# zhouyou-gu/sig-sdp-mmw

Hardware: AMD Instinct MI355X
Metric: mmw_iterations_per_sec (higher is better)
Workload: dtype f32

## Files before the change

### sig_sdp_mmw_amd/csrc/kernels_mfma.h

```cpp
#pragma once
#include "kernels_expm.h"

namespace mmw {

typedef short mf_s4 __attribute__((ext_vector_type(4)));
typedef short mf_s8 __attribute__((ext_vector_type(8)));
typedef __bf16 mf_bf8 __attribute__((ext_vector_type(8)));
typedef float mf_f16 __attribute__((ext_vector_type(16)));

__device__ __forceinline__ unsigned short bf16_rn(float x) { return __builtin_bit_cast(unsigned short, (__bf16)x); }
__device__ __forceinline__ float bf16_f32(unsigned short h) { return __uint_as_float((unsigned)h << 16); }
__device__ __forceinline__ unsigned split_bf16(float x) {
    const unsigned short hi = bf16_rn(x);
    const unsigned short lo = bf16_rn(x - bf16_f32(hi));
    return ((unsigned)hi << 16) | (unsigned)lo;
}

__global__ __launch_bounds__(BLOCK) void k_split_planes(size_t n4, const float4* __restrict__ src, uint2* __restrict__ hi, uint2* __restrict__ lo) {
    for (size_t o = (size_t)blockIdx.x * BLOCK + threadIdx.x; o < n4; o += (size_t)gridDim.x * BLOCK) {
        const float4 x = src[o];
        const unsigned a = split_bf16(x.x), b = split_bf16(x.y), c = split_bf16(x.z), d = split_bf16(x.w);
        hi[o] = make_uint2((a >> 16) | (b & 0xFFFF0000u), (c >> 16) | (d & 0xFFFF0000u));
        lo[o] = make_uint2((a & 0xFFFFu) | (b << 16), (c & 0xFFFFu) | (d << 16));
    }
}

constexpr double SDM_FX = 1099511627776.0;
constexpr int MF_KROWS = 16;
constexpr int MF_UNION_ROWS = 640;
constexpr int MF_KPAD = 4;
struct MfmaDev {
    int nb;
    const int* desc;
    const int* un_fixed;
    const int* order;
    const int* kbase;
    const unsigned* afrag;
};
struct MfEpi {
    const float* F = nullptr;
    const float* X2 = nullptr;
    float c3 = 0.f;
    unsigned short* out_planes = nullptr;
    unsigned short* y_planes = nullptr;
    long long* dfx = nullptr;
    double* tr_part = nullptr;
};
template <int MT, int GT, int KC, int PL = 2, int AP = 2> constexpr int mf_chunk_bytes() { return KC * (1024 * PL * GT + 1024 * AP * MT); }
template <int MT, int GT, int KC, int NB, int PL = 2, int AP = 2> constexpr int mf_lds_bytes() { return MF_UNION_ROWS * 4 + 64 * 4 + NB * mf_chunk_bytes<MT, GT, KC, PL, AP>(); }
constexpr bool mf_first(int mode) { return mode == SPMM_FIRST || mode == SPMM_FIRST16; }
constexpr int mf_planes(int mode) { return mf_first(mode) ? 1 : 2; }
constexpr int mf_apieces(int mode) { return mode == SPMM_FIRST16 ? 1 : 2; }
typedef _Float16 mf_h8 __attribute__((ext_vector_type(8)));
constexpr float MF_F16_SCALE = 1048576.0f;
__device__ __forceinline__ unsigned short f16_rn(float x) { return __builtin_bit_cast(unsigned short, (_Float16)x); }
__device__ __forceinline__ float f16_f32(unsigned short h) { return (float)__builtin_bit_cast(_Float16, h); }
__device__ __forceinline__ unsigned split_f16_scaled(float x) {
    const float xs = x * MF_F16_SCALE;
    const unsigned short hi = f16_rn(xs);
    const unsigned short lo = f16_rn(xs - f16_f32(hi));
    return ((unsigned)hi << 16) | (unsigned)lo;
}
__device__ __forceinline__ size_t mf_pos16(int w) {
    const int j = (w & 3) + 4 * ((w >> 8) & 1), lane = (w >> 2) & 63;
    return ((size_t)(w >> 9) * 64 + lane) * 8 + j;
}
__global__ __launch_bounds__(BLOCK) void k_plane_f16(size_t n4, const float4* __restrict__ src, uint2* __restrict__ dst) {
    for (size_t o = (size_t)blockIdx.x * BLOCK + threadIdx.x; o < n4; o += (size_t)gridDim.x * BLOCK) {
        const float4 x = src[o];
        dst[o] = make_uint2((unsigned)f16_rn(x.x) | ((unsigned)f16_rn(x.y) << 16), (unsigned)f16_rn(x.z) | ((unsigned)f16_rn(x.w) << 16));
    }
}


__device__ __forceinline__ void mf_wait_vmcnt(int n) {
    switch (n) {
#define MMW_W(N) case N: asm volatile("s_waitcnt vmcnt(" #N ")" ::: "memory"); break;
        MMW_W(0) MMW_W(1) MMW_W(2) MMW_W(3) MMW_W(4) MMW_W(5) MMW_W(6) MMW_W(7) MMW_W(8) MMW_W(9) MMW_W(10) MMW_W(11) MMW_W(12)
        MMW_W(13) MMW_W(14) MMW_W(15) MMW_W(16) MMW_W(17) MMW_W(18) MMW_W(19) MMW_W(20) MMW_W(21) MMW_W(22) MMW_W(23) MMW_W(24)
        MMW_W(25) MMW_W(26) MMW_W(27) MMW_W(28) MMW_W(29) MMW_W(30) MMW_W(31) MMW_W(32) MMW_W(33) MMW_W(34) MMW_W(35) MMW_W(36)
        MMW_W(37) MMW_W(38) MMW_W(39) MMW_W(40) MMW_W(41) MMW_W(42) MMW_W(43) MMW_W(44) MMW_W(45) MMW_W(46) MMW_W(47) MMW_W(48)
#undef MMW_W
        default: asm volatile("s_waitcnt vmcnt(0)" ::: "memory"); break;
    }
}

__device__ __forceinline__ int mf_div(int n, int d, float rd) { (void)d; return (int)(((float)n + 0.5f) * rd); }
__device__ __forceinline__ void mf_dma16(const char* src, unsigned lds) {
    asm volatile("s_mov_b32 m0, %1\n\ts_nop 0\n\tglobal_load_lds_dwordx4 %0, off" : : "v"(src), "s"(lds) : "memory", "m0");
}

template <int MODE, int MT, int NT, int NW, int MS, int KC, int NB>
__global__ __launch_bounds__(NW * 64)
void k_spmm_mfma(MfmaDev M, int Dpad, size_t plane_bytes, const char* __restrict__ Upl, const float* __restrict__ U,
                 float* __restrict__ Out, double ascale_d, double shift_d, double* __restrict__ partial, double* __restrict__ partial_o2,
                 const ExpmPlan* __restrict__ plan, int step, int* __restrict__ viol, unsigned long long* __restrict__ stamps, MfEpi E) {
    static_assert(MODE == SPMM_PLAIN || MODE == SPMM_LANCZOS || MODE == SPMM_AXPBY || mf_first(MODE), "the matrix-core SpMM has the plain, the Lanczos, the AXPBY and the first-order epilogue");
    static_assert(MF_KPAD % KC == 0, "the fragment image pads a block's k-steps to whole chunks");
    constexpr bool F16 = mf_first(MODE);
    constexpr bool A16 = MODE == SPMM_FIRST16;
    constexpr int AP = mf_apieces(MODE), AB = 1024 * AP;
    unsigned long long tk0 = 0, tk1 = 0, acc_wait = 0, acc_issue = 0, acc_comp = 0, t_pro = 0;
    if (stamps) tk0 = __builtin_amdgcn_s_memtime();
    typedef __attribute__((address_space(3))) void* lds_vp;
    typedef const __attribute__((address_space(1))) void* glb_vp;
    constexpr int THREADS = NW * 64;
    bool shifted = false;
    if (plan) {
        if (MODE == SPMM_LANCZOS) {
            if (step > plan_steps(plan, step - 1)) return;
            shifted = plan->apost != 0 && partial_o2 != nullptr;
            if (shifted) shift_d = plan->mu;
        } else if (F16) {
            shift_d = plan->mu;
        } else if (step > plan->m) return;
        if (!(A16 ? plan->f16a_ok : (F16 ? plan->f16_ok : plan->mfma_ok)) && viol && blockIdx.x == 0 && blockIdx.y == 0 && threadIdx.x == 0) atomicOr(viol, VIOL_OPERANDS);
    }
    const float ascale = (float)ascale_d, shift = (float)shift_d;
    static_assert(NW % MS == 0 && MT % MS == 0, "row tiles and waves split evenly");
    constexpr int NWN = NW / MS;
    constexpr int MTW = MT / MS;
    constexpr int GT = NWN * NT;
    constexpr int PL = mf_planes(MODE);
    constexpr int CHUNK = mf_chunk_bytes<MT, GT, KC, PL, AP>();
    constexpr int B1 = 1024 * PL * GT;
    constexpr int A_OFF = KC * B1;
    extern __shared__ __attribute__((aligned(16))) char smem_raw[];
    int* un_l = reinterpret_cast<int*>(smem_raw);
    int* orow_l = reinterpret_cast<int*>(smem_raw + MF_UNION_ROWS * 4);
    char* bufs = smem_raw + MF_UNION_ROWS * 4 + 64 * 4;
    const unsigned bufs_l = (unsigned)(size_t)(lds_vp)bufs;

    const int per = (M.nb + 7) >> 3;
    const int rb = (blockIdx.x & 7) * per + (blockIdx.x >> 3);
    if (rb >= M.nb) return;
    const int col0 = blockIdx.y * (GT * 32);
    const int ng = min(GT, (Dpad - col0) >> 5);
    const int spr = ng * 4;
    const int* dsc = M.desc + (size_t)rb * 8;
    const int q0 = dsc[0], nrows = dsc[1];
    const int kb = M.kbase[rb];
    const int KS = M.kbase[rb + 1] - kb;
    const int NC = KS / KC;
    const int lane = threadIdx.x & 63;
    const int wv = __builtin_amdgcn_readfirstlane(threadIdx.x >> 6);
    const int wm = wv / NWN, wn = wv - wm * NWN;

    for (int i = threadIdx.x; i < KS * MF_KROWS; i += THREADS) un_l[i] = M.un_fixed[(size_t)rb * MF_UNION_ROWS + i];
    if ((int)threadIdx.x < 64) orow_l[threadIdx.x] = (int)threadIdx.x < nrows ? M.order[q0 + threadIdx.x] : -1;

    const int rmode = (ng & 3) == 0 ? 2 : ((ng & 3) == 2 ? 1 : 0);
    auto rot = [&](int q) { return rmode == 2 ? q : (rmode == 1 ? (q >> 1) : 0); };

    constexpr int NJ = (KC * (PL * GT + AP * MT) + NW - 1) / NW;
    const int nB1 = PL * ng, nP1 = nB1 + AP * MT, nI = KC * nP1;
    const int cw = wv < nI ? (nI - wv + NW - 1) / NW : 0;
    const char* pbase[NJ];
    unsigned pmul[NJ];
    int prow[NJ], pdst[NJ];
    const unsigned pitch = (unsigned)Dpad * 2u;
    const char* afr = reinterpret_cast<const char*>(M.afrag) + (size_t)kb * (AB * MT);
    const float rP1 = 1.0f / (float)nP1, rspr = 1.0f / (float)spr;
#pragma unroll
    for (int j = 0; j < NJ; ++j) {
        const int i = wv + NW * j;
        const int kk = mf_div(i, nP1, rP1), i1 = i - kk * nP1;
        pbase[j] = Upl;
        pmul[j] = 0;
        prow[j] = 0;
        pdst[j] = 0;
        if (i < nI && i1 < nB1) {
            const int slot = i1 * 64 + lane;
            const int p = (PL == 2 && slot >= MF_KROWS * spr) ? 1 : 0, rem = slot - p * (MF_KROWS * spr);
            const int r = mf_div(rem, spr, rspr), t = rem - r * spr;
            int G = (t >> 2) - rot(r & 3);
            if (G < 0) G += ng;
            pbase[j] = Upl + ((size_t)p * plane_bytes + (size_t)col0 * 2u + (size_t)(G * 4 + (t & 3)) * 16u);
            pmul[j] = pitch;
            prow[j] = kk * MF_KROWS + r;
            pdst[j] = kk * B1 + i1 * 1024;
        } else if (i < nI) {
            pbase[j] = afr + (kk * (AB * MT) + (i1 - nB1) * 1024 + lane * 16);
            pdst[j] = A_OFF + kk * (AB * MT) + (i1 - nB1) * 1024;
        }
        pdst[j] = __builtin_amdgcn_readfirstlane(pdst[j]);
    }
    auto issue = [&](int c) {
        const unsigned dst_l = bufs_l + (unsigned)((c % NB) * CHUNK);
        const unsigned astep = (unsigned)c * (unsigned)(KC * AB * MT);
#pragma unroll
        for (int j = 0; j < NJ; ++j) {
            if (j < cw) {
                const char* src = pbase[j] + ((size_t)(unsigned)un_l[c * (KC * MF_KROWS) + prow[j]] * pmul[j] + (pmul[j] ? 0u : astep));
                mf_dma16(src, dst_l + (unsigned)pdst[j]);
            }
        }
    };

    const int g16 = lane >> 4, l16 = lane & 15, tq = l16 >> 2, tp = l16 & 3;
    unsigned rbase[NT];
    bool tile_on[NT];
#pragma unroll
    for (int i = 0; i < NT; ++i) {
        const int G = wn * NT + i;
        tile_on[i] = G < ng;
        int Gp = (tile_on[i] ? G : 0) + rot(tq);
        if (Gp >= ng) Gp -= ng;
        rbase[i] = (unsigned)((8 * (g16 >> 1) + tq) * spr * 16 + Gp * 64 + (g16 & 1) * 32 + tp * 8);
    }
    const unsigned row4 = (unsigned)(4 * spr * 16), plane_l = (unsigned)(MF_KROWS * spr * 16);

    mf_f16 acc[MTW][NT];
#pragma unroll
    for (int m = 0; m < MTW; ++m)
#pragma unroll
        for (int i = 0; i < NT; ++i)
#pragma unroll
            for (int v = 0; v < 16; ++v) acc[m][i][v] = 0.f;

    __syncthreads();
#pragma unroll
    for (int c = 0; c < NB - 1; ++c)
        if (c < NC) issue(c);
    if (stamps) { tk1 = __builtin_amdgcn_s_memtime(); t_pro = tk1 - tk0; }
    for (int c = 0; c < NC; ++c) {
        const int younger = min(NC - 1 - c, NB - 2);
        mf_wait_vmcnt(cw * younger);
        __builtin_amdgcn_s_barrier();
        if (stamps) { const unsigned long long t = __builtin_amdgcn_s_memtime(); acc_wait += t - tk1; tk1 = t; }
        if (c + NB - 1 < NC) issue(c + NB - 1);
        if (stamps) { const unsigned long long t = __builtin_amdgcn_s_memtime(); acc_issue += t - tk1; tk1 = t; }
        const char* cb = bufs + (c % NB) * CHUNK;
#pragma unroll
        for (int kk = 0; kk < KC; ++kk) {
            const char* bb = cb + kk * B1;
            mf_s8 ahi[MTW], alo[MTW];
#pragma unroll
            for (int m = 0; m < MTW; ++m) {
                const char* af = cb + A_OFF + (kk * MT + wm * MTW + m) * AB + lane * 16;
                const uint4 a0 = *reinterpret_cast<const uint4*>(af);
                if constexpr (A16) {
                    ahi[m] = __builtin_bit_cast(mf_s8, a0);
                    alo[m] = ahi[m];
                    continue;
                }
                const uint4 a1 = *reinterpret_cast<const uint4*>(af + 1024);
                const unsigned w[8] = {a0.x, a0.y, a0.z, a0.w, a1.x, a1.y, a1.z, a1.w};
                unsigned h[4], l[4];
#pragma unroll
                for (int i = 0; i < 4; ++i) {
                    h[i] = __builtin_amdgcn_perm(w[2 * i + 1], w[2 * i], 0x07060302u);
                    l[i] = __builtin_amdgcn_perm(w[2 * i + 1], w[2 * i], 0x05040100u);
                }
                const uint4 hv = make_uint4(h[0], h[1], h[2], h[3]), lv = make_uint4(l[0], l[1], l[2], l[3]);
                ahi[m] = __builtin_bit_cast(mf_s8, hv);
                alo[m] = __builtin_bit_cast(mf_s8, lv);
            }
#pragma unroll
            for (int i = 0; i < NT; ++i) {
                typedef __attribute__((address_space(3))) mf_s4* lp;
                const char* p0 = bb + rbase[i];
                const mf_s4 h0 = __builtin_amdgcn_ds_read_tr16_b64_v4i16((lp)(p0));
                const mf_s4 h1 = __builtin_amdgcn_ds_read_tr16_b64_v4i16((lp)(p0 + row4));
                if constexpr (F16) {
                    const mf_s8 bh = {h0[0], h0[1], h0[2], h0[3], h1[0], h1[1], h1[2], h1[3]};
#pragma unroll
                    for (int m = 0; m < MTW; ++m) {
                        if constexpr (!A16) acc[m][i] = __builtin_amdgcn_mfma_f32_32x32x16_f16(__builtin_bit_cast(mf_h8, alo[m]), __builtin_bit_cast(mf_h8, bh), acc[m][i], 0, 0, 0);
                        acc[m][i] = __builtin_amdgcn_mfma_f32_32x32x16_f16(__builtin_bit_cast(mf_h8, ahi[m]), __builtin_bit_cast(mf_h8, bh), acc[m][i], 0, 0, 0);
                    }
                } else {
                    const mf_s4 l0 = __builtin_amdgcn_ds_read_tr16_b64_v4i16((lp)(p0 + plane_l));
                    const mf_s4 l1 = __builtin_amdgcn_ds_read_tr16_b64_v4i16((lp)(p0 + plane_l + row4));
                    const mf_s8 bhi = {h0[0], h0[1], h0[2], h0[3], h1[0], h1[1], h1[2], h1[3]};
                    const mf_s8 blo = {l0[0], l0[1], l0[2], l0[3], l1[0], l1[1], l1[2], l1[3]};
#pragma unroll
                    for (int m = 0; m < MTW; ++m) {
                        acc[m][i] = __builtin_amdgcn_mfma_f32_32x32x16_bf16(__builtin_bit_cast(mf_bf8, alo[m]), __builtin_bit_cast(mf_bf8, bhi), acc[m][i], 0, 0, 0);
                        acc[m][i] = __builtin_amdgcn_mfma_f32_32x32x16_bf16(__builtin_bit_cast(mf_bf8, ahi[m]), __builtin_bit_cast(mf_bf8, blo), acc[m][i], 0, 0, 0);
                        acc[m][i] = __builtin_amdgcn_mfma_f32_32x32x16_bf16(__builtin_bit_cast(mf_bf8, ahi[m]), __builtin_bit_cast(mf_bf8, bhi), acc[m][i], 0, 0, 0);
                    }
                }
            }
        }
        if (stamps) { const unsigned long long t = __builtin_amdgcn_s_memtime(); acc_comp += t - tk1; tk1 = t; }
    }

    if constexpr (F16) {
        const int h2 = lane >> 5, cl = lane & 31;
        const float emu = Out ? (float)exp(shift_d) : 1.f;
        float* red = reinterpret_cast<float*>(bufs);
        float* rowred = red + MS * GT * 32;
        static_assert((MS * GT * 32 + NWN * 32 * MT) * 4 <= NB * CHUNK, "the epilogue's reductions fit into the chunk buffers");
        float rn[MTW][16], d2t[NT];
#pragma unroll
        for (int m = 0; m < MTW; ++m)
#pragma unroll
            for (int v = 0; v < 16; ++v) rn[m][v] = 0.f;
#pragma unroll
        for (int i = 0; i < NT; ++i) {
            if (!tile_on[i]) continue;
            const int col = col0 + (wn * NT + i) * 32 + cl;
            float dot2 = 0.f;
#pragma unroll
            for (int m = 0; m < MTW; ++m) {
                int rows[16];
                float u[16], yy[16];
#pragma unroll
                for (int v = 0; v < 16; ++v) rows[v] = orow_l[32 * (wm * MTW + m) + (v & 3) + 8 * (v >> 2) + 4 * h2];
#pragma unroll
                for (int v = 0; v < 16; ++v) u[v] = U[(size_t)max(rows[v], 0) * Dpad + col];
#pragma unroll
                for (int v = 0; v < 16; ++v) {
                    const float o = ascale * acc[m][i][v] - shift * u[v];
                    const float y = u[v] + o;
                    yy[v] = 0.f;
                    if (rows[v] >= 0) {
                        dot2 += o * o;
                        yy[v] = y * y;
                        if (Out) Out[(size_t)rows[v] * Dpad + col] = y * emu;
                    }
                    const unsigned w = split_bf16(y);
                    const unsigned wp = dpp_u32<DPP_QUAD_XOR1>(w);
                    if (rows[v] >= 0) {
                        const unsigned val = (cl & 1) ? ((wp & 0xFFFFu) | (w << 16)) : ((w >> 16) | (wp & 0xFFFF0000u));
                        unsigned short* g = E.y_planes + (size_t)rows[v] * Dpad * 2 + (size_t)(col >> 5) * 64 + ((cl & 1) ? 32 : 0) + (col & 30);
                        *reinterpret_cast<unsigned*>(g) = val;
                    }
                }
#pragma unroll
                for (int v = 0; v < 16; ++v) rn[m][v] += group_sum(yy[v], 32);
            }
            float a, b;
            rows32(dot2, a, b);
            d2t[i] = a + b;
        }
        __syncthreads();
#pragma unroll
        for (int i = 0; i < NT; ++i)
            if (tile_on[i] && h2 == 0) red[(wm * GT + wn * NT + i) * 32 + cl] = d2t[i];
        if (cl == 0) {
#pragma unroll
            for (int m = 0; m < MTW; ++m)
#pragma unroll
                for (int v = 0; v < 16; ++v) rowred[wn * (32 * MT) + 32 * (wm * MTW + m) + (v & 3) + 8 * (v >> 2) + 4 * h2] = rn[m][v];
        }
        __syncthreads();
        for (int t = threadIdx.x; t < ng * 32; t += THREADS) {
            float d2 = 0.f;
#pragma unroll
            for (int g = 0; g < MS; ++g) d2 += red[g * GT * 32 + t];
            partial_o2[(size_t)rb * Dpad + col0 + t] = (double)d2;
        }
        if (wv == 0) {
            double s = 0.0;
            if (lane < nrows) {
                float f = 0.f;
#pragma unroll
                for (int g = 0; g < NWN; ++g) f += rowred[g * (32 * MT) + lane];
                s = (double)f;
                atomicAdd(reinterpret_cast<unsigned long long*>(E.dfx) + orow_l[lane], (unsigned long long)__double2ll_rn(s * SDM_FX));
            }
            s = wave_sum(s);
            if (lane == 0) E.tr_part[(size_t)blockIdx.y * gridDim.x + blockIdx.x] = s;
        }
        if (stamps && lane == 0) {
            const unsigned long long te = __builtin_amdgcn_s_memtime();
            unsigned long long* o = stamps + ((size_t)(blockIdx.y * gridDim.x + blockIdx.x) * NW + wv) * 8;
            o[0] = t_pro; o[1] = acc_wait; o[2] = acc_issue; o[3] = acc_comp; o[4] = te - tk0; o[5] = (unsigned long long)NC; o[6] = tk0; o[7] = te - tk1;
        }
        return;
    }
    const int h2 = lane >> 5, cl = lane & 31;
#pragma unroll
    for (int i = 0; i < NT; ++i) {
        if (!tile_on[i]) continue;
        const int col = col0 + (wn * NT + i) * 32 + cl;
        float dot = 0.f, dot2 = 0.f;
#pragma unroll
        for (int m = 0; m < MTW; ++m) {
            int rows[16];
            float u[16];
#pragma unroll
            for (int v = 0; v < 16; ++v) rows[v] = orow_l[32 * (wm * MTW + m) + (v & 3) + 8 * (v >> 2) + 4 * h2];
            float x2[16];
            if (MODE == SPMM_LANCZOS) {
#pragma unroll
                for (int v = 0; v < 16; ++v) u[v] = U[(size_t)max(rows[v], 0) * Dpad + col];
            }
            if (MODE == SPMM_AXPBY) {
#pragma unroll
                for (int v = 0; v < 16; ++v) {
                    u[v] = E.F[(size_t)max(rows[v], 0) * Dpad + col];
                    x2[v] = E.X2[(size_t)max(rows[v], 0) * Dpad + col];
                }
            }
#pragma unroll
            for (int v = 0; v < 16; ++v) {
                float o;
                if (MODE == SPMM_LANCZOS) {
                    o = ascale * acc[m][i][v] - shift * u[v];
                    if (rows[v] >= 0) {
                        dot += u[v] * o;
                        dot2 += o * o;
                    }
                } else if (MODE == SPMM_AXPBY) {
                    o = ascale * acc[m][i][v] + shift * u[v] + E.c3 * x2[v];
                } else {
                    o = ascale * acc[m][i][v];
                }
                if (rows[v] >= 0) {
                    const size_t at = (size_t)rows[v] * Dpad + col;
                    Out[at] = o;
                    if (MODE != SPMM_LANCZOS && E.out_planes) {
                        const unsigned w = split_bf16(o);
                        E.out_planes[at] = (unsigned short)(w >> 16);
                        *reinterpret_cast<unsigned short*>(reinterpret_cast<char*>(E.out_planes) + plane_bytes + at * 2) = (unsigned short)(w & 0xFFFFu);
                    }
                }
            }
        }
        if (MODE == SPMM_LANCZOS) {
            float a, b;
            rows32(dot, a, b);
            const float d1 = a + b;
            rows32(dot2, a, b);
            const float d2 = a + b;
            if (MS == 1) {
                if (h2 == 0) {
                    partial[(size_t)rb * Dpad + col] = (double)d1;
                    if (shifted) partial_o2[(size_t)rb * Dpad + col] = (double)d2;
                }
            } else if (h2 == 0) {
                float* red = reinterpret_cast<float*>(bufs);
                red[((wm * GT + wn * NT + i) * 32 + cl) * 2] = d1;
                red[((wm * GT + wn * NT + i) * 32 + cl) * 2 + 1] = d2;
            }
        }
    }
    if (MODE == SPMM_LANCZOS && MS > 1) {
        __syncthreads();
        const float* red = reinterpret_cast<const float*>(bufs);
        for (int t = threadIdx.x; t < ng * 32; t += THREADS) {
            float d1 = 0.f, d2 = 0.f;
#pragma unroll
            for (int g = 0; g < MS; ++g) {
                d1 += red[((g * GT) * 32 + t) * 2];
                d2 += red[((g * GT) * 32 + t) * 2 + 1];
            }
            partial[(size_t)rb * Dpad + col0 + t] = (double)d1;
            if (shifted) partial_o2[(size_t)rb * Dpad + col0 + t] = (double)d2;
        }
    }
    if (stamps && lane == 0) {
        const unsigned long long te = __builtin_amdgcn_s_memtime();
        unsigned long long* o = stamps + ((size_t)(blockIdx.y * gridDim.x + blockIdx.x) * NW + wv) * 8;
        o[0] = t_pro; o[1] = acc_wait; o[2] = acc_issue; o[3] = acc_comp; o[4] = te - tk0; o[5] = (unsigned long long)NC; o[6] = tk0; o[7] = te - tk1;
    }
}


struct SdMfmaDev {
    const int* tbase;
    const int* tptr;
    const unsigned short* trc;
    const unsigned short* tmask;
    int nedges;
};
constexpr int SDM_GT = 4;
constexpr int SDM_KC = 2;
template <int MT> constexpr int sdm_rows() { return 32 * MT + 32 * SDM_GT; }
template <int MT> constexpr int sdm_chunk_bytes() { return 2 * sdm_rows<MT>() * 32 * SDM_KC; }
template <int MT, int NB = 2> constexpr int sdm_lds_bytes() { return sdm_rows<MT>() * 4 + NB * sdm_chunk_bytes<MT>(); }

constexpr int FV_COLS = 8;
constexpr double F16_SUBNORMAL_ROW = 640.0 * 2.842170943040401e-14;
struct FirstVerify {
    ExpmPlan* plan = nullptr;
    int* viol = nullptr;
    const double* o2 = nullptr;
    const double* u2 = nullptr;
    const double* du2 = nullptr;
    int rows = 0;
    int n_o2 = 0, n_u2 = 0, Dpad = 0;
    int nwg = 0;
    double cA = 0.0;
    double du_scale = 1.0;
};
__device__ inline void first_verify(const FirstVerify& V, int wg) {
    __shared__ double shv[3 * FV_COLS][16];
    const int BLOCK_V = (int)blockDim.x, NWV = BLOCK_V >> 6;
    const int c0 = wg * FV_COLS;
    const int lane = threadIdx.x & 63, wv = threadIdx.x >> 6, q8 = lane & 7, sl = lane >> 3;
    double a_o2 = 0.0, a_u2 = 0.0, a_du = 0.0;
    for (int b = wv * 8 + sl; b < V.n_o2; b += NWV * 8) a_o2 += V.o2[(size_t)b * V.Dpad + c0 + q8];
    for (int b = wv * 8 + sl; b < V.n_u2; b += NWV * 8) {
        a_u2 += V.u2[(size_t)b * V.Dpad + c0 + q8];
        if (V.du2) a_du += V.du2[(size_t)b * V.Dpad + c0 + q8];
    }
    a_o2 = stride_sum(a_o2, 8);
    a_u2 = stride_sum(a_u2, 8);
    a_du = stride_sum(a_du, 8);
    if (lane < FV_COLS) { shv[lane][wv] = a_o2; shv[FV_COLS + lane][wv] = a_u2; shv[2 * FV_COLS + lane][wv] = a_du; }
    __syncthreads();
    if (threadIdx.x < 64) {
        double e = 0.0, et = 0.0;
        if (threadIdx.x < FV_COLS) {
            const int q = (int)threadIdx.x;
            double o2 = 0.0, u2 = 0.0, du2 = 0.0;
            for (int w = 0; w < NWV; ++w) { o2 += shv[q][w]; u2 += shv[FV_COLS + q][w]; du2 += shv[2 * FV_COLS + q][w]; }
            if (u2 > 0.0) {
                const double rho = V.plan->rho, absn = V.plan->absn;
                et = first_order_bound(sqrt(o2 / u2), rho);
                if (!V.du2) du2 = F16_UNIT * F16_UNIT * u2 + (double)V.rows * 8.881784197001252e-16;
                e = et + exp(rho) * (absn * (V.du_scale * sqrt(du2 / u2) + V.cA) + F16_SUBNORMAL_ROW);
            }
            if (!(e >= 0.0)) e = et = 1e300;
        }
        const double best = wave_max(e), best_t = wave_max(et);
        if (threadIdx.x == 0) {
            auto up = [](double x) {
                float f = (float)x;
                if (!(f >= 0.0f)) f = __uint_as_float(0x7f800000u);
                if ((double)f < x) f = __uint_as_float(__float_as_uint(f) + 1u);
                return __float_as_uint(f);
            };
            atomicMax(&V.plan->conv[1], up(best));
            atomicMax(&V.plan->first_est, up(best_t));
            if (wg == 0) V.plan->m_eff = 1;
            if (!(best <= V.plan->tol) || !V.plan->apost || V.plan->nsub != 1 || V.plan->overflow) atomicOr(V.viol, VIOL_FIRST);
        }
    }
}
__global__ __launch_bounds__(BLOCK) void k_first_verify(FirstVerify V) { first_verify(V, (int)blockIdx.x); }

template <int MT, int NB = 2>
__global__ __launch_bounds__(4 * MT * 64)
void k_sddmm_mfma(MfmaDev M, SdMfmaDev S, int K, int Dpad, const char* __restrict__ Ypl, const float* __restrict__ d,
                  const double* __restrict__ tr_part, int ntr, float* __restrict__ xs_val, float* __restrict__ xs_avg, int accumulate,
                  long long* __restrict__ rsfx = nullptr , const long long* __restrict__ dfx = nullptr,
                  unsigned long long* __restrict__ stamps = nullptr ,
                  FirstVerify V = FirstVerify{}) {
    {
        const int nbx = ((M.nb + 7) >> 3) << 3;
        if ((int)blockIdx.x >= nbx) {
            if (!V.plan) return;
            const int nfv = 8 * (int)gridDim.y;
            for (int cg = ((int)blockIdx.x - nbx) + 8 * (int)blockIdx.y; cg < V.nwg; cg += nfv) {
                first_verify(V, cg);
                __syncthreads();
            }
            return;
        }
    }
    unsigned long long tk0 = 0, tk1 = 0, acc_wait = 0, acc_issue = 0, acc_comp = 0, t_pro = 0, t_red = 0, t_store = 0;
    if (stamps) tk0 = __builtin_amdgcn_s_memtime();
    const int by = (int)blockIdx.y;
    constexpr int NW = 4 * MT, THREADS = NW * 64;
    constexpr int RA = 32 * MT, R = sdm_rows<MT>();
    constexpr int CHUNK = sdm_chunk_bytes<MT>();
    constexpr int NP = R / 8;
    constexpr int NJ = (NP + NW - 1) / NW;
    typedef __attribute__((address_space(3))) void* lds_vp;
    extern __shared__ __attribute__((aligned(16))) char smem_raw[];
    int* rows_l = reinterpret_cast<int*>(smem_raw);
    char* bufs = smem_raw + R * 4;
    const unsigned bufs_l = (unsigned)(size_t)(lds_vp)bufs;
    __shared__ double sh_tr[NW];

    const int per = (M.nb + 7) >> 3;
    const int rb = (blockIdx.x & 7) * per + (blockIdx.x >> 3);
    if (rb >= M.nb) return;
    const int* dsc = M.desc + (size_t)rb * 8;
    const int q0 = dsc[0], nrows = dsc[1], nun = dsc[5];
    const int ntile = (nun + 31) >> 5;
    const int ut0 = dsc[6] + by * SDM_GT;
    if (ut0 >= ntile) return;
    const int lane = threadIdx.x & 63;
    const int wv = __builtin_amdgcn_readfirstlane(threadIdx.x >> 6);
    const int wm = wv >> 2, wn = wv & 3;

    double tsum = 0.0;
    for (int i = threadIdx.x; i < ntr; i += THREADS) tsum += tr_part[i];
    tsum = wave_sum(tsum);
    if (lane == 0) sh_tr[wv] = tsum;
    for (int i = threadIdx.x; i < R; i += THREADS) {
        int g;
        if (i < RA) g = M.order[q0 + min(i, nrows - 1)];
        else g = M.un_fixed[(size_t)rb * MF_UNION_ROWS + min(ut0 * 32 + (i - RA), MF_UNION_ROWS - 1)];
        rows_l[i] = g;
    }
    __syncthreads();
    double tr = 0.0;
#pragma unroll
    for (int w = 0; w < NW; ++w) tr += sh_tr[w];
    tr /= (double)K;
    int tw0 = 0, tw1 = 0;
    unsigned mk = 0u;
    if (ut0 + wn < ntile) {
        const int t = S.tbase[rb] + (ut0 + wn) * MT + wm;
        tw0 = S.tptr[t];
        tw1 = S.tptr[t + 1];
        if (rsfx) mk = (unsigned)S.tmask[(size_t)t * 64 + lane];
    }

    const unsigned pitch = (unsigned)Dpad * 4u;
    const char* pbase[NJ];
#pragma unroll
    for (int j = 0; j < NJ; ++j) {
        const int i = wv + NW * j;
        pbase[j] = Ypl;
        if (i < NP) {
            const int row = 8 * i + (lane >> 3), pos = lane & 7;
            const int slot = (pos - (row >> 1)) & 7;
            pbase[j] = Ypl + ((size_t)(unsigned)rows_l[row] * pitch + (size_t)slot * 16u);
        }
    }
    const int cw = wv < NP ? (NP - wv + NW - 1) / NW : 0;
    auto issue = [&](int c) {
        const unsigned dst_l = bufs_l + (unsigned)((c % NB) * CHUNK);
#pragma unroll
        for (int j = 0; j < NJ; ++j)
            if (j < cw) mf_dma16(pbase[j] + (size_t)c * (64 * SDM_KC), dst_l + (unsigned)((wv + NW * j) * 1024));
    };
    const int r = lane & 31, h = lane >> 5;
    const int ra = 32 * wm + r, rbw = RA + 32 * wn + r;
    unsigned offA[SDM_KC][2], offB[SDM_KC][2];
#pragma unroll
    for (int kk = 0; kk < SDM_KC; ++kk)
#pragma unroll
        for (int p = 0; p < 2; ++p) {
            offA[kk][p] = (unsigned)(ra * 128 + (((4 * p + 2 * kk + h) + (ra >> 1)) & 7) * 16);
            offB[kk][p] = (unsigned)(rbw * 128 + (((4 * p + 2 * kk + h) + (rbw >> 1)) & 7) * 16);
        }
    mf_f16 acc;
#pragma unroll
    for (int v = 0; v < 16; ++v) acc[v] = 0.f;
    const int NC = Dpad / (16 * SDM_KC);
#pragma unroll
    for (int c = 0; c < NB - 1; ++c)
        if (c < NC) issue(c);
    if (stamps) { tk1 = __builtin_amdgcn_s_memtime(); t_pro = tk1 - tk0; }
    for (int c = 0; c < NC; ++c) {
        mf_wait_vmcnt(cw * min(NC - 1 - c, NB - 2));
        __builtin_amdgcn_s_barrier();
        if (stamps) { const unsigned long long t = __builtin_amdgcn_s_memtime(); acc_wait += t - tk1; tk1 = t; }
        if (c + NB - 1 < NC) issue(c + NB - 1);
        if (stamps) { const unsigned long long t = __builtin_amdgcn_s_memtime(); acc_issue += t - tk1; tk1 = t; }
        const char* cb = bufs + (c % NB) * CHUNK;
#pragma unroll
        for (int kk = 0; kk < SDM_KC; ++kk) {
            const uint4 ah = *reinterpret_cast<const uint4*>(cb + offA[kk][0]);
            const uint4 al = *reinterpret_cast<const uint4*>(cb + offA[kk][1]);
            const uint4 bh = *reinterpret_cast<const uint4*>(cb + offB[kk][0]);
            const uint4 bl = *reinterpret_cast<const uint4*>(cb + offB[kk][1]);
            acc = __builtin_amdgcn_mfma_f32_32x32x16_bf16(__builtin_bit_cast(mf_bf8, al), __builtin_bit_cast(mf_bf8, bh), acc, 0, 0, 0);
            acc = __builtin_amdgcn_mfma_f32_32x32x16_bf16(__builtin_bit_cast(mf_bf8, ah), __builtin_bit_cast(mf_bf8, bl), acc, 0, 0, 0);
            acc = __builtin_amdgcn_mfma_f32_32x32x16_bf16(__builtin_bit_cast(mf_bf8, ah), __builtin_bit_cast(mf_bf8, bh), acc, 0, 0, 0);
        }
        if (stamps) { const unsigned long long t = __builtin_amdgcn_s_memtime(); acc_comp += t - tk1; tk1 = t; }
    }
    static_assert(NW * 4096 + 4 * 32 * MT * 4 <= NB * CHUNK, "tiles and row-sum parts fit into the chunk buffers");
    constexpr int EPL = 4;
    unsigned rc[EPL];
    float xa[EPL];
    auto fetch_list = [&](int base) {
#pragma unroll
        for (int k = 0; k < EPL; ++k) {
            const int w = base + k * 64 + lane;
            rc[k] = w < tw1 ? (unsigned)S.trc[w] : 0xFFFFu;
            xa[k] = (w < tw1 && accumulate) ? xs_avg[w] : 0.f;
        }
    };
    fetch_list(tw0);
    float rsv[16];
    float csum = 0.f;
    if (rsfx) {
#pragma unroll
        for (int v = 0; v < 16; ++v) {
            const float m = ((mk >> v) & 1u) ? acc[v] : 0.f;
            csum += m;
            rsv[v] = group_sum(m, 32);
        }
        float ca, cb;
        rows32(csum, ca, cb);
        csum = ca + cb;
    }
    if (stamps) { const unsigned long long t = __builtin_amdgcn_s_memtime(); t_red = t - tk1; tk1 = t; }
    __syncthreads();
    float* rsl = reinterpret_cast<float*>(bufs) + NW * 1024;
    if (rsfx && (lane & 31) == 0) {
#pragma unroll
        for (int v = 0; v < 16; ++v) rsl[wn * RA + 32 * wm + (v & 3) + 8 * (v >> 2) + 4 * (lane >> 5)] = rsv[v];
    }
    float* tile = reinterpret_cast<float*>(bufs) + wv * 1024;
#pragma unroll
    for (int v = 0; v < 16; ++v) tile[((v & 3) + 8 * (v >> 2) + 4 * h) * 32 + r] = acc[v];
    if (rsfx) __syncthreads();
    else {
        __builtin_amdgcn_fence(__ATOMIC_ACQ_REL, "wavefront");
        __builtin_amdgcn_wave_barrier();
    }
    const float inv_tr = (float)(1.0 / tr);
    for (int base = tw0; base < tw1; base += 64 * EPL) {
        if (base != tw0) fetch_list(base);
#pragma unroll
        for (int k = 0; k < EPL; ++k)
            if (rc[k] != 0xFFFFu) {
                const int w = base + k * 64 + lane;
                const float x = tile[rc[k]] * inv_tr;
                xs_val[w] = x;
                if (accumulate) xs_avg[w] = xa[k] + x;
            }
    }
    if (rsfx && lane < 32 && csum != 0.f) {
        const long long q = __double2ll_rn((double)csum / tr * SDM_FX);
        atomicAdd(reinterpret_cast<unsigned long long*>(rsfx) + rows_l[RA + 32 * wn + lane], (unsigned long long)q);
    }
    if (by == 0)
        for (int i = threadIdx.x; i < nrows; i += THREADS) {
            const int row = rows_l[i];
            const float x = (float)((dfx ? (double)dfx[row] * (1.0 / SDM_FX) : (double)d[row]) / tr);
            xs_val[S.nedges + row] = x;
            if (accumulate) xs_avg[S.nedges + row] += x;
        }
    if (rsfx)
        for (int i = threadIdx.x; i < nrows; i += THREADS) {
            const float sum4 = ((rsl[i] + rsl[RA + i]) + rsl[2 * RA + i]) + rsl[3 * RA + i];
            const long long q = __double2ll_rn((double)sum4 / tr * SDM_FX);
            atomicAdd(reinterpret_cast<unsigned long long*>(rsfx) + rows_l[i], (unsigned long long)q);
        }
    if (stamps && lane == 0) {
        const unsigned long long te = __builtin_amdgcn_s_memtime();
        t_store = te - tk1;
        unsigned long long* o = stamps + ((size_t)(blockIdx.y * gridDim.x + blockIdx.x) * NW + wv) * 8;
        o[0] = t_pro; o[1] = acc_wait; o[2] = acc_issue; o[3] = acc_comp; o[4] = te - tk0; o[5] = t_red; o[6] = tk0; o[7] = t_store;
    }
}

}
```

Before: 6639.

## Transpose epilogue tiles through LDS for vectorized plane and output stores

Reworks the MFMA epilogue so each wave stages its 32x32 result tile in a padded LDS buffer, transposes it so each lane owns a contiguous row segment, and then writes the bf16 hi/lo planes and the Out matrix with 16-byte vector stores. This replaces the per-element scattered 4-byte stores and DPP shuffles. Row-norm reductions are computed from the transposed data rather than with per-element group sums. It also uses 32-bit byte offsets and skips masking work for fully populated row tiles. The cost is extra LDS traffic, wave barriers, and reuse of the chunk buffers for staging.

```diff
diff --git a/sig_sdp_mmw_amd/csrc/kernels_mfma.h b/sig_sdp_mmw_amd/csrc/kernels_mfma.h
--- a/sig_sdp_mmw_amd/csrc/kernels_mfma.h
+++ b/sig_sdp_mmw_amd/csrc/kernels_mfma.h
@@ -291,59 +291,105 @@
         const float emu = Out ? (float)exp(shift_d) : 1.f;
         float* red = reinterpret_cast<float*>(bufs);
         float* rowred = red + MS * GT * 32;
-        static_assert((MS * GT * 32 + NWN * 32 * MT) * 4 <= NB * CHUNK, "the epilogue's reductions fit into the chunk buffers");
-        float rn[MTW][16], d2t[NT];
-#pragma unroll
-        for (int m = 0; m < MTW; ++m)
-#pragma unroll
-            for (int v = 0; v < 16; ++v) rn[m][v] = 0.f;
+        constexpr int MF_YP = 36;
+        float* ytile = rowred + NWN * 32 * MT + wv * (32 * MF_YP);
+        static_assert(((MS * GT * 32 + NWN * 32 * MT) + NW * 32 * MF_YP) * 4 <= NB * CHUNK, "the epilogue's reductions and one staged tile per wave fit into the chunk buffers");
+        static_assert((MS * GT * 32 + NWN * 32 * MT) % 4 == 0 && MF_YP % 4 == 0, "staged rows are read 16 bytes at a time");
+        const unsigned dp4 = (unsigned)Dpad * 4u;
+        const char* Ub = reinterpret_cast<const char*>(U);
+        float d2t[NT];
 #pragma unroll
         for (int i = 0; i < NT; ++i) {
+            d2t[i] = 0.f;
             if (!tile_on[i]) continue;
-            const int col = col0 + (wn * NT + i) * 32 + cl;
+            const unsigned colb = (unsigned)(col0 + (wn * NT + i) * 32 + cl) * 4u;
             float dot2 = 0.f;
 #pragma unroll
             for (int m = 0; m < MTW; ++m) {
+                const int left = nrows - 32 * (wm * MTW + m);
+                if (left <= 0) continue;
                 int rows[16];
-                float u[16], yy[16];
+                float u[16];
 #pragma unroll
                 for (int v = 0; v < 16; ++v) rows[v] = orow_l[32 * (wm * MTW + m) + (v & 3) + 8 * (v >> 2) + 4 * h2];
-#pragma unroll
-                for (int v = 0; v < 16; ++v) u[v] = U[(size_t)max(rows[v], 0) * Dpad + col];
+                if (left >= 32) {
+#pragma unroll
+                    for (int v = 0; v < 16; ++v) u[v] = *reinterpret_cast<const float*>(Ub + ((unsigned)rows[v] * dp4 + colb));
+                } else {
+#pragma unroll
+                    for (int v = 0; v < 16; ++v) u[v] = *reinterpret_cast<const float*>(Ub + ((unsigned)max(rows[v], 0) * dp4 + colb));
+#pragma unroll
+                    for (int v = 0; v < 16; ++v) u[v] = rows[v] >= 0 ? u[v] : 0.f;
+                }
 #pragma unroll
                 for (int v = 0; v < 16; ++v) {
-                    const float o = ascale * acc[m][i][v] - shift * u[v];
-                    const float y = u[v] + o;
-                    yy[v] = 0.f;
-                    if (rows[v] >= 0) {
-                        dot2 += o * o;
-                        yy[v] = y * y;
-                        if (Out) Out[(size_t)rows[v] * Dpad + col] = y * emu;
-                    }
-                    const unsigned w = split_bf16(y);
-                    const unsigned wp = dpp_u32<DPP_QUAD_XOR1>(w);
-                    if (rows[v] >= 0) {
-                        const unsigned val = (cl & 1) ? ((wp & 0xFFFFu) | (w << 16)) : ((w >> 16) | (wp & 0xFFFF0000u));
-                        unsigned short* g = E.y_planes + (size_t)rows[v] * Dpad * 2 + (size_t)(col >> 5) * 64 + ((cl & 1) ? 32 : 0) + (col & 30);
-                        *reinterpret_cast<unsigned*>(g) = val;
-                    }
-                }
-#pragma unroll
-                for (int v = 0; v < 16; ++v) rn[m][v] += group_sum(yy[v], 32);
+                    const float o = __builtin_fmaf(ascale, acc[m][i][v], -(shift * u[v]));
+                    acc[m][i][v] = u[v] + o;
+                    dot2 = __builtin_fmaf(o, o, dot2);
+                }
             }
             float a, b;
             rows32(dot2, a, b);
             d2t[i] = a + b;
+            if (NT > 1) __builtin_amdgcn_sched_barrier(0);
         }
         __syncthreads();
 #pragma unroll
         for (int i = 0; i < NT; ++i)
             if (tile_on[i] && h2 == 0) red[(wm * GT + wn * NT + i) * 32 + cl] = d2t[i];
-        if (cl == 0) {
-#pragma unroll
-            for (int m = 0; m < MTW; ++m)
-#pragma unroll
-                for (int v = 0; v < 16; ++v) rowred[wn * (32 * MT) + 32 * (wm * MTW + m) + (v & 3) + 8 * (v >> 2) + 4 * h2] = rn[m][v];
+#pragma unroll
+        for (int m = 0; m < MTW; ++m) {
+            const int left = nrows - 32 * (wm * MTW + m);
+            if (left <= 0) continue;
+            const int row = orow_l[32 * (wm * MTW + m) + cl];
+            const unsigned rowb = (unsigned)max(row, 0) * dp4;
+            float rn = 0.f;
+#pragma unroll
+            for (int i = 0; i < NT; ++i) {
+                if (!tile_on[i]) continue;
+#pragma unroll
+                for (int v = 0; v < 16; ++v) ytile[((v & 3) + 8 * (v >> 2) + 4 * h2) * MF_YP + cl] = acc[m][i][v];
+                __builtin_amdgcn_fence(__ATOMIC_ACQ_REL, "wavefront");
+                __builtin_amdgcn_wave_barrier();
+                float y[16];
+#pragma unroll
+                for (int k = 0; k < 4; ++k) {
+                    const float4 q = *reinterpret_cast<const float4*>(ytile + cl * MF_YP + 16 * h2 + 4 * k);
+                    y[4 * k] = q.x; y[4 * k + 1] = q.y; y[4 * k + 2] = q.z; y[4 * k + 3] = q.w;
+                }
+                __builtin_amdgcn_fence(__ATOMIC_ACQ_REL, "wavefront");
+                __builtin_amdgcn_wave_barrier();
+                float s = 0.f;
+#pragma unroll
+                for (int k = 0; k < 16; ++k) s = __builtin_fmaf(y[k], y[k], s);
+                float a, b;
+                rows32(s, a, b);
+                rn += a + b;
+                unsigned hi[8], lo[8];
+#pragma unroll
+                for (int k = 0; k < 8; ++k) {
+                    const unsigned w0 = split_bf16(y[2 * k]), w1 = split_bf16(y[2 * k + 1]);
+                    hi[k] = (w0 >> 16) | (w1 & 0xFFFF0000u);
+                    lo[k] = (w0 & 0xFFFFu) | (w1 << 16);
+                }
+                const unsigned tcol = (unsigned)(col0 + (wn * NT + i) * 32);
+                auto store = [&]() {
+                    char* g = reinterpret_cast<char*>(E.y_planes) + (rowb + (tcol * 4u + (unsigned)h2 * 32u));
+                    *reinterpret_cast<uint4*>(g) = make_uint4(hi[0], hi[1], hi[2], hi[3]);
+                    *reinterpret_cast<uint4*>(g + 16) = make_uint4(hi[4], hi[5], hi[6], hi[7]);
+                    *reinterpret_cast<uint4*>(g + 64) = make_uint4(lo[0], lo[1], lo[2], lo[3]);
+                    *reinterpret_cast<uint4*>(g + 80) = make_uint4(lo[4], lo[5], lo[6], lo[7]);
+                    if (Out) {
+                        char* og = reinterpret_cast<char*>(Out) + (rowb + (tcol * 4u + (unsigned)h2 * 64u));
+#pragma unroll
+                        for (int k = 0; k < 4; ++k)
+                            *reinterpret_cast<float4*>(og + 16 * k) = make_float4(y[4 * k] * emu, y[4 * k + 1] * emu, y[4 * k + 2] * emu, y[4 * k + 3] * emu);
+                    }
+                };
+                if (left >= 32) store();
+                else if (row >= 0) store();
+            }
+            if (h2 == 0) rowred[wn * (32 * MT) + 32 * (wm * MTW + m) + cl] = rn;
         }
         __syncthreads();
         for (int t = threadIdx.x; t < ng * 32; t += THREADS) {
```

Result: no change. 6661 (median of 6 runs) (+0.3%).
